# vicpc00/td-vc-gan

Hardware: AMD Instinct MI355X
Metric: audio-seconds/sec (G+D train step, stage-1) (higher is better)
Workload: dtype f32 (fp32 storage and accumulation everywhere; FiLM cond_var.2 forward and weight-grad as split-bf16 x6 products -- three exact bf16 pieces per operand, six piece products on the bf16 MFMA, fp32 accumulate: fp32-level accuracy; every other kernel exact-fp32 MFMA)

## Files before the change

### td-vc-gan_amd/csrc/conv_common.h

```cpp
#pragma once
#include <hip/hip_runtime.h>
#include <stdint.h>
#include <mutex>

#define TDVC_BIG_LDS_ONCE(k)                                                                                         \
  do {                                                                                                               \
    static std::once_flag f_;                                                                                        \
    std::call_once(f_, [&] { hipFuncSetAttribute(reinterpret_cast<const void*>(k), hipFuncAttributeMaxDynamicSharedMemorySize, 160 * 1024); }); \
  } while (0)
namespace tdvc {
extern int g_trace_on;
extern int g_force_tile;
extern int g_force_gemm_tile;
extern int g_force_generic;
extern int g_lds_cap;
extern int g_knob[9];
void trace_kernel(const void* fn);
}
#define TDVC_TRACE(k) do { if (tdvc::g_trace_on) tdvc::trace_kernel(reinterpret_cast<const void*>(k)); } while (0)

namespace tdvc {

enum { MODE_DIRECT = 0, MODE_DOWN = 1, MODE_UP = 2 };
enum { XF_NONE = 0, XF_LRELU = 1, XF_FILM_LRELU = 2, XF_MASK_LRELU = 3, XF_MASK_TANH = 4 };
enum { EPI_FWD = 0, EPI_MASK = 1, EPI_FILM = 2, EPI_PLAIN = 3 };
enum { POST_NONE = 0, POST_LRELU = 1, POST_TANH = 2 };

struct Xf {
  int kind; float slope; float scale;
  const float* aux; long aux_bs;
};

struct Opnd {
  const float* p; long bs; int T; int Cg; Xf xf;
};

struct GemmConvP {
  Opnd x;
  const float* w; long w_sg, w_sm, w_sc; int K; int tap_flip;
  int mode, s, d, pad, reflect, J;
  int R, Cred, Cc, N, groups, lo, span, XS, WS;
  int i0;
  int mirror_pad;
  int stage_rows;
  int chan_stage;
  int w_nat;
  int w_packed;
  float* y; long y_bs; int Ty; int Cy_g;
  int epi;
  const float* bias;
  const float* bias3;
  const float* res; long res_bs;
  int post; float post_slope; float out_scale;
  const float* add; long add_bs; float add_scale;
  const float* mx; long mx_bs; float m_slope;
  const float* gb; long gb_bs; float* dgb; long dgb_bs;
};

struct WgradP {
  Opnd a;
  Opnd x;
  int mode, s, d, pad, reflect, J, K;
  int R, Cred, N, groups, lo, span, NTc, XS, AS;
  int i0;
  int ntiles;
  float* slab; long slab_stride;
  long w_sg, w_sm, w_sc;
};

// ... 51 lines not shown
__device__ __forceinline__ void tile_commit(const RegTile<NV>& t, const RegTile<NV>* a, const RegTile<NV>* c, const Xf& xf,
                                            float* dst, int XS, int nvalid, int nrows, int span, int ebase, int tid) {
  typedef float f32x2_t __attribute__((ext_vector_type(2)));
  const int nvec = span >> 2, total = nrows * nvec;
  const float inv = 1.0f / (float)nvec;
  const int kind = xf.kind;
  const float sl = xf.slope, sc = xf.scale;
#pragma unroll
  for (int i = 0; i < NV; ++i) {
    const int e = ebase + tid + i * 256;
    if (e >= total) continue;
    const int r = (int)(((float)e + 0.5f) * inv);
    const int vv = e - r * nvec;
    f32x4_t val = t.v[i];
    if (r < nvalid) {
      if (kind == XF_LRELU) {
#pragma unroll
        for (int q = 0; q < 4; ++q) val[q] = fmaxf(val[q], val[q] * sl);
      } else if (kind == XF_FILM_LRELU) {
#pragma unroll
        for (int q = 0; q < 4; ++q) { const float h = val[q] * (1.f + a->v[i][q]) + c->v[i][q]; val[q] = fmaxf(h, h * sl); }
      } else if (kind == XF_MASK_LRELU) {
#pragma unroll
        for (int q = 0; q < 4; ++q) val[q] = a->v[i][q] > 0.f ? val[q] : val[q] * sl;
      } else if (kind == XF_MASK_TANH) {
#pragma unroll
        for (int q = 0; q < 4; ++q) val[q] = val[q] * (1.f - a->v[i][q] * a->v[i][q]);
      }
      if (sc != 1.f) {
#pragma unroll
        for (int q = 0; q < 4; ++q) val[q] *= sc;
      }
    }
    f32x2_t* d2 = reinterpret_cast<f32x2_t*>(dst + r * XS + 4 * vv);
    d2[0] = (f32x2_t){val[0], val[1]};
    d2[1] = (f32x2_t){val[2], val[3]};
  }
}

typedef __amdgpu_buffer_rsrc_t srd_t;
typedef unsigned int u32x4_t __attribute__((ext_vector_type(4)));

__device__ __forceinline__ srd_t make_srd(const float* base, int bytes) {
  const uintptr_t a = reinterpret_cast<uintptr_t>(base);
  const unsigned lo = __builtin_amdgcn_readfirstlane((unsigned)(a & 0xffffffffu));
  const unsigned hi = __builtin_amdgcn_readfirstlane((unsigned)(a >> 32));
  const int nb = __builtin_amdgcn_readfirstlane(bytes > 0 ? bytes : 0);
  float* ub = reinterpret_cast<float*>(((uintptr_t)hi << 32) | lo);
  return __builtin_amdgcn_make_buffer_rsrc(ub, 0, nb, 0x00020000);
}
__device__ __forceinline__ f32x4_t buf_load4(srd_t rs, int voff) {
  return __builtin_bit_cast(f32x4_t, __builtin_amdgcn_raw_buffer_load_b128(rs, voff, 0, 0));
}

template <int NV>
__device__ __forceinline__ void tile_issue(RegTile<NV>& t, const float* base, int rowstride, int nvalid, int nrows, int span,
                                           int cvalid, int ebase, int tid, int vlo, int vhi) {
  const int nvec = span >> 2, total = nrows * nvec;
  const float inv = 1.0f / (float)nvec;
  const srd_t rs = make_srd(base, nvalid > 0 ? ((nvalid - 1) * rowstride + cvalid) * 4 : 0);
#pragma unroll
  for (int i = 0; i < NV; ++i) {
    const int e = ebase + tid + i * 256;
    const int r = (int)(((float)e + 0.5f) * inv);
    const int vv = e - r * nvec;
    t.v[i] = buf_load4(rs, (e < total && r < nvalid && 4 * vv < cvalid && vv >= vlo && vv < vhi) ? (r * rowstride + 4 * vv) * 4 : 0x7f000000);
  }
}

struct RowWalk { int voff, loff, gstep, lstep, nk; bool active; };

__device__ __forceinline__ int walk_opaque(int n) { asm volatile("" : "+s"(n)); return n; }

__device__ __forceinline__ RowWalk make_walk(int tid, int nvec, int rp, int rowstride, int ls, int q0, int T) {
  RowWalk w;
  const int rsub = (int)(((float)tid + 0.5f) * (1.0f / (float)nvec));
  const int vv = tid - rsub * nvec;
  const int q = q0 + 4 * vv;
  w.active = rsub < rp;
  w.voff = (w.active && q >= 0 && q < T) ? (rsub * rowstride + q) * 4 : 0x7f000000;
  w.nk = T - q < 4 ? T - q : 4;
  w.loff = rsub * ls + 4 * vv;
  w.gstep = rp * rowstride * 4;
  w.lstep = rp * ls;
  return w;
}

template <int NP>
__device__ __forceinline__ void walk_issue(RegTile<NP>& t, srd_t rs, const RowWalk& w, int np) {
  int vo = w.voff;
#pragma unroll
  for (int i = 0; i < NP; ++i) {
    if (i < walk_opaque(np)) { t.v[i] = buf_load4(rs, vo); vo += w.gstep; }
  }
}

template <int NP>
__device__ __forceinline__ void walk_commit_act(RegTile<NP>& t, const RowWalk& w, int np, float* lds, float slope, float scale, bool tail = false) {
  if (!w.active) return;
  const int base = w.loff;
#pragma unroll
  for (int i = 0; i < NP; ++i) {
    if (i < walk_opaque(np)) {
      f32x4_t o;
#pragma unroll
      for (int q = 0; q < 4; ++q) { const float v = t.v[i][q]; o[q] = fmaxf(v, v * slope); }
// ... 144 lines not shown
```

### td-vc-gan_amd/csrc/conv_lean.h

```cpp
#pragma once
#include <hip/hip_runtime.h>

namespace tdvc {

enum { LXF_ACT = 0, LXF_FILM = 1, LXF_MASK_LRELU = 2, LXF_MASK_TANH = 3, LXF_COND = 4 };

struct LeanP {
  const float* x; const float* w; float* y;
  const float* bias; const float* bias3; const float* res; const float* add;
  const float* aux;
  const float* mx; const float* gb; float* dgb;
  int x_bs, y_bs, res_bs, add_bs, aux_bs, mx_bs, gb_bs, dgb_bs;
  int T, Cin, Cout, Cw, K, d, pad, flip, reflect, mirror;
  int Cc, span, lo, i0, XS, WS;
  int xrp, xnp, wrp, wnp;
  int post;
  const float* cw; const float* k3; float* cv0;
  int cw_stride, Cv, cv0_bs, ES;
  unsigned* sbits; const unsigned* mbits;
  int sb_bs, mb_bs;
  int swz;
  int one_ahead;
  int fold, seg, Bn;
  int vec;
  float slope, in_scale, out_scale, add_scale, m_slope;
};

hipError_t launch_conv_lean(LeanP p, int B, int xfk, int epi, hipStream_t st);
hipError_t launch_conv_lean_cond(LeanP p, int B, hipStream_t st);

}
```

### td-vc-gan_amd/csrc/conv_lean.hip

```cpp
#include "conv_common.h"
#include "conv_lean.h"

PROF_DEFINE(tdvc_debug_lean_prof)

namespace tdvc {

typedef float f32x4 __attribute__((ext_vector_type(4)));




template <int XFK>
__device__ __forceinline__ float lean_xform(const LeanP& p, float v, int b, int c, int q) {
  if (XFK == LXF_ACT) { v = fmaxf(v, v * p.slope); }
  else {
    const float* a = p.aux + (long)b * p.aux_bs + (long)c * p.T + q;
    if (XFK == LXF_FILM) { const float h = v * (1.f + a[0]) + a[(long)p.Cin * p.T]; v = fmaxf(h, h * p.slope); }
    else if (XFK == LXF_MASK_LRELU) { v = a[0] > 0.f ? v : v * p.slope; }
    else { v = v * (1.f - a[0] * a[0]); }
  }
  return v * p.in_scale;
}

template <int XFK>
__device__ __forceinline__ float lean_fetch(const LeanP& p, int b, int c, int q) {
  if (p.reflect) { if (q < 0) q = -q; else if (q >= p.T) q = 2 * (p.T - 1) - q; }
  if (q < 0 || q >= p.T) return 0.f;
  return lean_xform<XFK>(p, p.x[(long)b * p.x_bs + (long)c * p.T + q], b, c, q);
}

#ifndef LEAN_OCC_SMALL
#define LEAN_OCC_SMALL 4
#endif
constexpr int lean_min_blocks(int m_rep, int n_rep, int wm, int xfk) {
  if (m_rep == 1 && n_rep == 4 && wm == 1 && xfk == LXF_ACT) return 5;
  return m_rep * n_rep >= 9 ? 2 : ((m_rep * n_rep >= 8 || (wm == 4 && xfk == LXF_FILM)) ? 3 : LEAN_OCC_SMALL);
}
#ifndef LEAN_RING_1
#define LEAN_RING_1 2
#endif
#ifndef LEAN_RING_2
#define LEAN_RING_2 2
#endif
constexpr int lean_ring_depth(int m_rep, int n_rep) { return m_rep * n_rep == 1 ? LEAN_RING_1 : (m_rep * n_rep == 2 ? LEAN_RING_2 : 0); }
template <int M_REP, int N_REP, int WM, int WN, int XFK, int EPI, bool FOLD = false>
__global__ __launch_bounds__(256, lean_min_blocks(M_REP, N_REP, WM, XFK)) void conv_lean_kernel(const LeanP p) {
  extern __shared__ __attribute__((aligned(16))) float smem[];
  constexpr int MT = 16 * M_REP * WM, NT = 16 * N_REP * WN;
  constexpr int XVP = (M_REP >= 9 || NT <= 64) ? 4 : (MT >= 32 ? 12 : 6);
  constexpr int WVP = MT >= 48 ? 10 : (MT >= 32 ? 6 : 4);
  float* xs = smem;
  float* ws = smem + p.xnp * p.xrp * p.XS;
  constexpr int WX = 25;
  float* es = ws + p.wnp * p.wrp * p.WS;
  float* wx = es + p.Cv * p.ES;

  const int tid = threadIdx.x, lane = tid & 63, wave = tid >> 6;
  const int wm = wave / WN, wn = wave % WN;
  const int ln = lane & 15, kq = lane >> 4;
  int bx = blockIdx.x, by = blockIdx.y, bz = blockIdx.z;
  if (p.swz) {
    const int gx = gridDim.x, gy = gridDim.y;
    const int nwg = gx * gy * gridDim.z;
    const int orig = bx + gx * (by + gy * bz);
    const int q = nwg >> 3, r = nwg & 7, xcd = orig & 7;
    const int wg = (xcd < r ? xcd * (q + 1) : r * (q + 1) + (xcd - r) * q) + (orig >> 3);
    by = wg % gy;
    const int t = wg / gy;
    bx = t % gx; bz = t / gx;
  }
  const int n0 = FOLD ? 0 : bx * NT, r0 = by * MT, b = FOLD ? bz * p.fold : bz;
  const int wcol0 = wn * 16 * N_REP, wrow0 = wm * 16 * M_REP;
  PROF_DECL

  f32x4 acc[M_REP][N_REP];
#pragma unroll
  for (int m = 0; m < M_REP; ++m)
#pragma unroll
    for (int n = 0; n < N_REP; ++n) acc[m][n] = (f32x4){0.f, 0.f, 0.f, 0.f};

  const int q0 = n0 + p.lo;
  const bool vec_ok = p.vec != 0;
  const bool interior = (XFK != LXF_COND) && (XFK == LXF_ACT || !p.reflect);
  const bool tail = (p.T & 3) != 0;
  const bool end_tile = q0 < 0 || q0 + p.span > p.T;
  const int jc = p.K * p.Cc;
  const float* xrow0 = p.x + (long)b * p.x_bs;
  const float* arow0 = (XFK != LXF_ACT && XFK != LXF_COND) ? p.aux + (long)b * p.aux_bs : nullptr;
  const float* wgrow = p.w + (long)r0 * p.Cw;
// ... 322 lines not shown
#pragma unroll
            for (int n = 0; n < N_REP; ++n) mbv[n] = mv[n] ? mb[n] : -(1 << 28);
            for (int j = 0; j < p.K; ++j) {
              const float* wp = w_lane + (p.flip ? p.K - 1 - j : j);
              const float* xp[N_REP]; bool ok[N_REP];
#pragma unroll
              for (int n = 0; n < N_REP; ++n) {
                const int idx = mbv[n] + j * p.d;
                ok[n] = (unsigned)idx < (unsigned)p.span;
                xp[n] = xs + kq * p.XS + (ok[n] ? idx : 0);
              }
              ring_run(csteps, [&](int slot) {
#pragma unroll
                for (int m = 0; m < M_REP; ++m) wv[slot][m] = wp[m * wrep];
#pragma unroll
                for (int n = 0; n < N_REP; ++n) { xv[slot][n] = *xp[n]; xp[n] += 4 * p.XS; }
                wp += 4 * p.K;
              }, [&](int slot) {
#pragma unroll
                for (int m = 0; m < M_REP; ++m)
#pragma unroll
                  for (int n = 0; n < N_REP; ++n)
                    acc[m][n] = __builtin_amdgcn_mfma_f32_16x16x4f32(ok[n] ? xv[slot][n] : 0.f, wv[slot][m], acc[m][n], 0, 0, 0);
              });
            }
            continue;
          }
        }
        for (int j = 0; j < p.K; ++j) {
          const float* wj = w_lane + (p.flip ? p.K - 1 - j : j);
          for (int cs = 0; cs < csteps; ++cs) {
            float wm_[M_REP], xm_[N_REP];
#pragma unroll
            for (int m = 0; m < M_REP; ++m) wm_[m] = wj[m * 16 * p.WS + cs * 4 * p.K];
#pragma unroll
            for (int n = 0; n < N_REP; ++n) {
              const int idx = mb[n] + j * p.d;
              const bool ok = mv[n] && idx >= 0 && idx < p.span;
              const float t = xs[(cs * 4 + kq) * p.XS + (ok ? idx : 0)];
              xm_[n] = ok ? t : 0.f;
            }
#pragma unroll
            for (int m = 0; m < M_REP; ++m)
#pragma unroll
              for (int n = 0; n < N_REP; ++n)
                acc[m][n] = __builtin_amdgcn_mfma_f32_16x16x4f32(xm_[n], wm_[m], acc[m][n], 0, 0, 0);
          }
        }
      }
    }
    PROF(5)
  }

  if (!vec_ok) {
#pragma unroll
    for (int m = 0; m < M_REP; ++m) {
      const int co = r0 + wrow0 + m * 16 + ln;
      if (co >= p.Cout) continue;
      const long ro = (long)co * p.T;
      const float bias = (EPI == EPI_FWD && p.bias) ? p.bias[co] : 0.f;
#pragma unroll
      for (int n = 0; n < N_REP; ++n) {
#pragma unroll
        for (int q = 0; q < 4; ++q) {
          const int t = n0 + wcol0 + n * 16 + kq * 4 + q;
          if (t >= p.T) continue;
          const long oi = ro + t;
          float v = acc[m][n][q];
          if (EPI == EPI_FWD) {
            v += bias;
            if (p.bias3) v += p.bias3[((long)b * p.Cout + co) * 3 + (t == 0 ? 0 : (t == p.T - 1 ? 2 : 1))];
            if (p.res) v += p.res[(long)b * p.res_bs + oi];
            if (p.post == POST_LRELU) v = fmaxf(v, v * p.m_slope);
            else if (p.post == POST_TANH) v = tanhf(v);
            v *= p.out_scale;
          } else if (EPI == EPI_MASK) {
            v = p.mx[(long)b * p.mx_bs + oi] > 0.f ? v : v * p.m_slope;
          } else if (EPI == EPI_FILM) {
            const float h = p.mx[(long)b * p.mx_bs + oi];
            const float* gp = p.gb + (long)b * p.gb_bs + oi;
            const float ga = gp[0], be = gp[(long)p.Cout * p.T];
            const float dh2 = (h * (1.f + ga) + be) > 0.f ? v : v * p.m_slope;
            float* dg = p.dgb + (long)b * p.dgb_bs + oi;
            dg[0] = dh2 * h; dg[(long)p.Cout * p.T] = dh2;
            v = dh2 * (1.f + ga);
          }
          if (p.add) v += p.add_scale * p.add[(long)b * p.add_bs + oi];
          p.y[(long)b * p.y_bs + oi] = v;
        }
      }
    }
    PROF(6)
    PROF_END
    return;
  }
  auto epi_store = [&](f32x4 v, const int co, const int t0, const float bias, const int b) -> f32x4 {
    const long oi = (long)co * p.T + t0;
    if (EPI == EPI_FWD) {
#pragma unroll
      for (int q = 0; q < 4; ++q) v[q] += bias;
      if (p.bias3) {
        const float* k3 = p.bias3 + ((long)b * p.Cout + co) * 3;
        const float mid = k3[1];
#pragma unroll
        for (int q = 0; q < 4; ++q) v[q] += mid;
        if (t0 == 0) v[0] += k3[0] - mid;
        if (t0 + 4 == p.T) v[3] += k3[2] - mid;
      }
      if (p.res) { const f32x4 r = *reinterpret_cast<const f32x4*>(p.res + (long)b * p.res_bs + oi); v += r; }
      if (p.post == POST_LRELU) {
#pragma unroll
        for (int q = 0; q < 4; ++q) v[q] = fmaxf(v[q], v[q] * p.m_slope);
      } else if (p.post == POST_TANH) {
#pragma unroll
        for (int q = 0; q < 4; ++q) v[q] = tanhf(v[q]);
      }
      v *= p.out_scale;
    } else if (EPI == EPI_MASK) {
      if (N_REP >= 2 && p.mbits) {
        const unsigned wbits = p.mbits[(long)b * p.mb_bs + (long)co * (p.T >> 5) + (t0 >> 5)] >> (t0 & 31);
#pragma unroll
        for (int q = 0; q < 4; ++q) v[q] = ((wbits >> q) & 1u) ? v[q] : v[q] * p.m_slope;
      } else {
        const f32x4 mm = *reinterpret_cast<const f32x4*>(p.mx + (long)b * p.mx_bs + oi);
#pragma unroll
        for (int q = 0; q < 4; ++q) v[q] = mm[q] > 0.f ? v[q] : v[q] * p.m_slope;
      }
    } else if (EPI == EPI_FILM) {
      const f32x4 h = *reinterpret_cast<const f32x4*>(p.mx + (long)b * p.mx_bs + oi);
      const float* gp = p.gb + (long)b * p.gb_bs + oi;
      const f32x4 ga = *reinterpret_cast<const f32x4*>(gp);
      const f32x4 be = *reinterpret_cast<const f32x4*>(gp + (long)p.Cout * p.T);
      f32x4 dga, dbe;
#pragma unroll
      for (int q = 0; q < 4; ++q) {
        const float h2 = h[q] * (1.f + ga[q]) + be[q];
        const float dh2 = h2 > 0.f ? v[q] : v[q] * p.m_slope;
        dga[q] = dh2 * h[q]; dbe[q] = dh2; v[q] = dh2 * (1.f + ga[q]);
      }
      float* dg = p.dgb + (long)b * p.dgb_bs + oi;
      *reinterpret_cast<f32x4*>(dg) = dga;
      *reinterpret_cast<f32x4*>(dg + (long)p.Cout * p.T) = dbe;
    }
    if (p.add) { const f32x4 a4 = *reinterpret_cast<const f32x4*>(p.add + (long)b * p.add_bs + oi); v += a4 * p.add_scale; }
    *reinterpret_cast<f32x4*>(p.y + (long)b * p.y_bs + oi) = v;
    return v;
  };
  auto sign_nibble = [](const f32x4& v, const int t0) -> unsigned {
    return ((v[0] > 0.f ? 1u : 0u) | (v[1] > 0.f ? 2u : 0u) | (v[2] > 0.f ? 4u : 0u) | (v[3] > 0.f ? 8u : 0u)) << (t0 & 31);
  };

#pragma unroll
  for (int m = 0; m < M_REP; ++m) {
    const int co = r0 + wrow0 + m * 16 + ln;
    if (co >= p.Cout) continue;
    float bias = 0.f;
    if (EPI == EPI_FWD && p.bias) bias = p.bias[co];
    unsigned sb_word = 0;
#pragma unroll
    for (int n = 0; n < N_REP; ++n) {
      int t0 = n0 + wcol0 + n * 16 + kq * 4, bb = b;
      if (FOLD) { const int sg = t0 / p.T; t0 -= sg * p.T; bb = b + sg; if (bb >= p.Bn) continue; }
      if (t0 >= p.T) continue;
      const f32x4 v = epi_store(acc[m][n], co, t0, bias, bb);
      if (EPI == EPI_FWD && N_REP >= 2 && p.sbits) {
        const unsigned h = sign_nibble(v, t0);
        sb_word = (n & 1) ? (sb_word | h) : h;
        if (n & 1) {
          unsigned w = sb_word;
          w |= (unsigned)__shfl_xor((int)w, 16);
          w |= (unsigned)__shfl_xor((int)w, 32);
          if (kq == 0) p.sbits[(long)b * p.sb_bs + (long)co * (p.T >> 5) + (t0 >> 5)] = w;
        }
      }
    }
  }
  PROF(6)
  PROF_END
}

static inline void walk_geometry(int rows, int nvec, int* rp, int* np) {
  *rp = nvec <= 256 ? 256 / nvec : 0;
  if (*rp > rows) *rp = rows;
  *np = *rp ? (rows + *rp - 1) / *rp : 1 << 20;
}

template <int M_REP, int N_REP, int WM, int WN, int XFK, int EPI, bool FOLD = false>
static hipError_t lean_launch3(const LeanP& p, int B, hipStream_t st) {
  constexpr int MT = 16 * M_REP * WM, NT = 16 * N_REP * WN;
  auto k = conv_lean_kernel<M_REP, N_REP, WM, WN, XFK, EPI, FOLD>;
  TDVC_BIG_LDS_ONCE(k); TDVC_TRACE(k);
  dim3 grid(FOLD ? 1 : (p.T + NT - 1) / NT, (p.Cout + MT - 1) / MT, FOLD ? (B + p.fold - 1) / p.fold : B);
  LeanP q = p; q.swz = g_knob[0] && (long)grid.x * grid.y * grid.z >= 16;
  q.one_ahead = g_knob[8] != 0;
  const size_t lds = (size_t)(p.xnp * p.xrp * p.XS + p.wnp * p.wrp * p.WS) * sizeof(float);
  hipLaunchKernelGGL(k, grid, dim3(256), lds, st, q);
  return hipGetLastError();
}

template <int M_REP, int N_REP, int WM, int WN>
static hipError_t lean_launch_fold(const LeanP& p, int B, int xfk, int epi, hipStream_t st) {
  if (xfk == LXF_ACT && epi == EPI_FWD) return lean_launch3<M_REP, N_REP, WM, WN, LXF_ACT, EPI_FWD, true>(p, B, st);
  if (xfk == LXF_ACT && epi == EPI_PLAIN) return lean_launch3<M_REP, N_REP, WM, WN, LXF_ACT, EPI_PLAIN, true>(p, B, st);
  if (xfk == LXF_MASK_LRELU && epi == EPI_PLAIN) return lean_launch3<M_REP, N_REP, WM, WN, LXF_MASK_LRELU, EPI_PLAIN, true>(p, B, st);
  return hipErrorNotSupported;
}

template <int M_REP, int N_REP, int WM, int WN>
static hipError_t lean_launch2(const LeanP& p, int B, int xfk, int epi, hipStream_t st) {
  if (xfk == LXF_ACT && epi == EPI_FWD) return lean_launch3<M_REP, N_REP, WM, WN, LXF_ACT, EPI_FWD>(p, B, st);
  if (xfk == LXF_FILM && epi == EPI_FWD) return lean_launch3<M_REP, N_REP, WM, WN, LXF_FILM, EPI_FWD>(p, B, st);
  if (xfk == LXF_ACT && epi == EPI_MASK) return lean_launch3<M_REP, N_REP, WM, WN, LXF_ACT, EPI_MASK>(p, B, st);
  if (xfk == LXF_ACT && epi == EPI_FILM) return lean_launch3<M_REP, N_REP, WM, WN, LXF_ACT, EPI_FILM>(p, B, st);
  if (xfk == LXF_ACT && epi == EPI_PLAIN) return lean_launch3<M_REP, N_REP, WM, WN, LXF_ACT, EPI_PLAIN>(p, B, st);
  if (xfk == LXF_MASK_LRELU && epi == EPI_PLAIN) return lean_launch3<M_REP, N_REP, WM, WN, LXF_MASK_LRELU, EPI_PLAIN>(p, B, st);
  return hipErrorNotSupported;
}

hipError_t launch_conv_lean_cond(LeanP p, int B, hipStream_t st) {
  if ((p.T & 3) || !p.vec || p.K != 3 || p.d != 1 || p.pad != 1 || p.Cv * 3 > 24) return hipErrorNotSupported;
  const int MT = p.Cout <= 32 ? 32 : 64, NT = 256;
  p.mirror = 0; p.flip = 0; p.reflect = 0;
  const int first = -p.pad;
  const int lo = -4;
  p.lo = lo; p.i0 = first - lo;
  p.span = ((NT + (p.K - 1) * p.d - p.pad - lo) + 3) / 4 * 4;
  p.XS = ((p.span + 15) / 32) * 32 + 16;
  p.ES = ((p.span + 15) / 16) * 16 + 4;
  int Cc = 32;
  auto geom = [&](int cc) {
    p.Cc = cc; p.WS = p.K * cc + 2;
    p.xrp = cc; p.xnp = 1;
    walk_geometry(MT, p.K * cc / 4, &p.wrp, &p.wnp);
    return (size_t)(cc * p.XS + p.wnp * p.wrp * p.WS + p.Cv * p.ES + cc * 25) * sizeof(float);
  };
  size_t lds = geom(Cc);
  if (lds > (size_t)(g_lds_cap > 0 ? g_lds_cap : 80 * 1024) || p.wnp > (MT >= 48 ? 10 : 6)) lds = geom(Cc = 16);
  dim3 grid((p.T + NT - 1) / NT, (p.Cout + MT - 1) / MT, B);
  p.swz = g_knob[0] && (long)grid.x * grid.y * grid.z >= 16;
  if (MT == 32) {
    auto k = conv_lean_kernel<2, 4, 1, 4, LXF_COND, EPI_FWD>;
    TDVC_BIG_LDS_ONCE(k); TDVC_TRACE(k);
    hipLaunchKernelGGL(k, grid, dim3(256), lds, st, p);
  } else {
    auto k = conv_lean_kernel<4, 4, 1, 4, LXF_COND, EPI_FWD>;
    TDVC_BIG_LDS_ONCE(k); TDVC_TRACE(k);
    hipLaunchKernelGGL(k, grid, dim3(256), lds, st, p);
  }
  return hipGetLastError();
}

hipError_t launch_conv_lean(LeanP p, int B, int xfk, int epi, hipStream_t st) {
  const bool combo = (xfk == LXF_ACT) || (xfk == LXF_FILM && epi == EPI_FWD) || (xfk == LXF_MASK_LRELU && epi == EPI_PLAIN);
  if (!combo) return hipErrorNotSupported;
  struct Cand { int MT, NT, cfg; };
  static const Cand cands[] = {{64, 256, 2}, {48, 256, 5}, {32, 256, 1}, {64, 64, 4}, {32, 64, 6}, {16, 256, 0}, {16, 64, 3}};
  static const Cand tall = {144, 64, 7};
  const int R = p.Cout;
  int MT = 16, NT = 64, cfg = 3;
  for (const Cand& c : cands) {
    if (c.MT > 16 && R <= 16) continue;
    if (c.MT > 32 && R <= 32) continue;
    if (c.MT == 48 && !(R % 64 != 0 && (R + 47) / 48 * 48 < (R + 63) / 64 * 64)) continue;
    if (c.MT == 64 && c.NT == 256 && (R % 64 != 0 && (R + 47) / 48 * 48 < (R + 63) / 64 * 64)) continue;
    if (c.NT == 256 && p.T <= 80) continue;
    const long blocks = (long)((R + c.MT - 1) / c.MT) * ((p.T + c.NT - 1) / c.NT) * B;
    MT = c.MT; NT = c.NT; cfg = c.cfg;
    if (blocks >= (c.cfg == 4 ? 1024 : 512)) break;
  }
  if ((long)p.Cin * p.K <= 48 && p.T > 80 && p.mirror == 0) { MT = 16; NT = 256; cfg = 0; }
  if ((long)p.Cin * p.K <= 224 && p.T > 80 && (R >= 128 || R == 32)) { MT = 16; NT = 256; cfg = 0; }
  if (g_force_tile >= 0) {
    for (const Cand& c : cands)
      if (c.cfg == g_force_tile) { MT = c.MT; NT = c.NT; cfg = c.cfg; }
    if (g_force_tile == tall.cfg) { MT = tall.MT; NT = tall.NT; cfg = tall.cfg; }
  }
  if (p.sbits || p.mbits) {
    if (!p.vec || (p.T & 31) || p.T <= 80) return hipErrorNotSupported;
    if (cfg == 3 || cfg == tall.cfg) { MT = 16; NT = 256; cfg = 0; }
  }
  const int first = -p.pad;
  int lo = -p.pad - p.mirror;
  lo = -(((-lo) + 3) / 4 * 4);
  const int hi = (p.K - 1) * p.d - p.pad + p.mirror;
  p.lo = lo; p.i0 = first - lo;
  p.span = ((NT + hi - lo) + 3) / 4 * 4;
  p.fold = 1; p.seg = 0; p.Bn = B;
  const bool fold_combo = (xfk == LXF_ACT && (epi == EPI_FWD || epi == EPI_PLAIN)) || (xfk == LXF_MASK_LRELU && epi == EPI_PLAIN);
  if (g_knob[4] == 0 && g_force_tile < 0 && NT == 64 && R >= 32 && (p.T == 16 || p.T == 32) && p.Cin % 16 == 0 && B >= 64 / p.T && p.vec && !p.reflect && p.mirror == 0 && fold_combo &&
      !p.sbits && !p.mbits && (!p.aux || p.aux_bs == p.x_bs) && (long)(64 / p.T) * p.x_bs < (1L << 28)) {
    p.fold = 64 / p.T;
    p.seg = ((p.T + hi - lo) + 3) / 4 * 4;
    p.span = p.fold * p.seg;
    const long nb64 = (long)((R + 63) / 64) * ((B + p.fold - 1) / p.fold);
    if (nb64 >= 1024) { MT = 64; cfg = 4; } else { MT = 32; cfg = 6; }
  }
  p.XS = ((p.span + 15) / 32) * 32 + 16;
  const int xvp = (MT >= 144 || NT <= 64) ? 4 : (MT >= 32 ? 12 : 6), wvp = MT >= 48 ? 10 : (MT >= 32 ? 6 : 4);
  const size_t lds_cap = g_lds_cap > 0 ? (size_t)g_lds_cap : (size_t)((cfg == 4 ? 40 : 52) * 1024);
  int Cc = 0;
  const int cc_cap = (MT == 16 && p.Cin >= 256) ? 64 : 32;
  for (int cc = 4; cc <= cc_cap && cc <= ((p.Cin + 3) / 4) * 4; cc += 4) {
    int xrp, xnp, wrp, wnp;
    walk_geometry(cc, p.span / 4, &xrp, &xnp);
    walk_geometry(MT, p.K * cc / 4, &wrp, &wnp);
    const size_t lds = (size_t)(xnp * xrp * p.XS + wnp * wrp * (p.K * cc + 2)) * 4;
    if (lds > lds_cap || wnp > wvp || (xfk == LXF_ACT && xnp > xvp)) continue;
    if (p.fold > 1 && p.Cin % cc) continue;
    Cc = cc; p.xrp = xrp; p.xnp = xnp; p.wrp = wrp; p.wnp = wnp;
  }
  if (!Cc) return hipErrorNotSupported;
  p.Cc = Cc;
  p.WS = p.K * Cc + 2;
  if (p.fold > 1) return cfg == 4 ? lean_launch_fold<1, 4, 4, 1>(p, B, xfk, epi, st) : lean_launch_fold<1, 2, 2, 2>(p, B, xfk, epi, st);
  switch (cfg) {
    case 0: return lean_launch2<1, 4, 1, 4>(p, B, xfk, epi, st);
    case 1: return lean_launch2<2, 4, 1, 4>(p, B, xfk, epi, st);
    case 2: return lean_launch2<4, 4, 1, 4>(p, B, xfk, epi, st);
    case 3: return lean_launch2<1, 1, 1, 4>(p, B, xfk, epi, st);
    case 5: return lean_launch2<3, 4, 1, 4>(p, B, xfk, epi, st);
    case 6: return lean_launch2<1, 2, 2, 2>(p, B, xfk, epi, st);
    case 7: return lean_launch2<9, 1, 1, 4>(p, B, xfk, epi, st);
    default: return lean_launch2<1, 4, 4, 1>(p, B, xfk, epi, st);
  }
}

}
```

### td-vc-gan_amd/csrc/misc_kernels.hip

```cpp
#include "../../include/tdvc.h"
#include "api_util.h"
#include "conv_common.h"
#include <math.h>
#include <stdlib.h>
#include <string.h>

static thread_local char g_err[256] = "";
int tdvc_fail(int code, const char* msg) {
  snprintf(g_err, sizeof(g_err), "%s", msg ? msg : "");
  return code;
}
extern "C" const char* tdvc_last_error(void) { return g_err; }
extern "C" int tdvc_version(void) { return 200; }

#include <cxxabi.h>
#include <mutex>
#include <set>
#include <string>
namespace tdvc {
int g_trace_on = 0;
int g_force_tile = -1;
int g_force_gemm_tile = -1;
int g_lds_cap = 0;
int g_knob[9] = {0, 0, 0, 0, 0, 0, 0, 0, 0};
static std::mutex g_trace_mu;
static std::set<std::string> g_trace_names;
void trace_kernel(const void* fn) {
  const char* mangled = hipKernelNameRefByPtr(fn, nullptr);
  std::string name;
  if (mangled) {
    int status = 0;
    char* dem = abi::__cxa_demangle(mangled, nullptr, nullptr, &status);
    name = (status == 0 && dem) ? dem : mangled;
    free(dem);
  } else {
    char buf[32]; snprintf(buf, sizeof(buf), "kernel@%p", fn); name = buf;
  }
  std::lock_guard<std::mutex> lk(g_trace_mu);
  g_trace_names.insert(name);
}
}
extern "C" void tdvc_debug_force_tile(int cfg) { tdvc::g_force_tile = cfg; }
extern "C" void tdvc_debug_force_gemm_tile(int cfg) { tdvc::g_force_gemm_tile = cfg; }
extern "C" void tdvc_debug_lds_cap(int bytes) { tdvc::g_lds_cap = bytes; }
extern "C" void tdvc_debug_knob(int which, int value) { if (which >= 0 && which < 9) tdvc::g_knob[which] = value; }
namespace tdvc {
__global__ __launch_bounds__(256) void poison_lds_kernel(unsigned word, int nwords, unsigned* sink) {
  extern __shared__ __attribute__((aligned(16))) float smem[];
  unsigned* u = reinterpret_cast<unsigned*>(smem);
  for (int i = threadIdx.x; i < nwords; i += 256) u[i] = word;
  __syncthreads();
  unsigned acc = 0;
  for (int i = threadIdx.x; i < nwords; i += 256) acc ^= u[i];
  if (acc == 0x12345u && sink) sink[0] = acc;
}
}
extern "C" int tdvc_debug_poison_lds(uint32_t word, void* stream) {
  auto k = tdvc::poison_lds_kernel;
  TDVC_BIG_LDS_ONCE(k);
  hipLaunchKernelGGL(k, dim3(4096), dim3(256), 80 * 1024, (hipStream_t)stream, (unsigned)word, 80 * 1024 / 4, (unsigned*)nullptr);
  TDVC_CHECK_LAUNCH();
  return TDVC_OK;
}
namespace tdvc { __global__ void pmc_marker_kernel(int*) {} }
extern "C" int tdvc_debug_marker(void* stream) {
  hipLaunchKernelGGL(tdvc::pmc_marker_kernel, dim3(1), dim3(64), 0, (hipStream_t)stream, (int*)nullptr);
  TDVC_CHECK_LAUNCH();
  return TDVC_OK;
}
extern "C" void tdvc_debug_trace(int on) {
  std::lock_guard<std::mutex> lk(tdvc::g_trace_mu);
  if (on == 1) tdvc::g_trace_names.clear();
  tdvc::g_trace_on = on ? 1 : 0;
}
extern "C" size_t tdvc_debug_trace_dump(char* buf, size_t cap) {
  std::lock_guard<std::mutex> lk(tdvc::g_trace_mu);
  std::string all;
  for (const std::string& n : tdvc::g_trace_names) { all += n; all += '\n'; }
  if (buf && cap) { const size_t n = all.size() < cap - 1 ? all.size() : cap - 1; memcpy(buf, all.data(), n); buf[n] = 0; }
  return all.size() + 1;
}

namespace {

__device__ __forceinline__ float wave_sum(float v) {
#pragma unroll
  for (int o = 32; o > 0; o >>= 1) v += __shfl_xor(v, o);
  return v;
}

__device__ __forceinline__ float block_sum(float v, float* sh ) {
  v = wave_sum(v);
  __syncthreads();
  if ((threadIdx.x & 63) == 0) sh[threadIdx.x >> 6] = v;
  __syncthreads();
  float r = 0.f;
  const int nw = (blockDim.x + 63) >> 6;
  for (int i = 0; i < nw; ++i) r += sh[i];
// ... 938 lines not shown
```

Baseline: 313.6.

## Batch epilogue loads through buffer descriptors and specialize epilogue variants

Rewrites the lean conv kernel epilogue so that each group of output rows issues all of its auxiliary loads (residual, mask, FiLM gamma/beta, add, bias) first, then computes. Out-of-range accesses go through raw buffer loads and stores with bounds-checked descriptors instead of per-element branches. The epilogue is instantiated at compile time for vector vs scalar, add, mask bits and post-activation, which removes runtime branches and extends the vectorised path to folded tiles. The previous epilogue remains available behind a new debug knob. In exchange, register pressure and code size go up, which could hurt occupancy.

```diff
diff --git a/td-vc-gan_amd/csrc/conv_common.h b/td-vc-gan_amd/csrc/conv_common.h
--- a/td-vc-gan_amd/csrc/conv_common.h
+++ b/td-vc-gan_amd/csrc/conv_common.h
@@ -14,7 +14,7 @@
 extern int g_force_gemm_tile;
 extern int g_force_generic;
 extern int g_lds_cap;
-extern int g_knob[9];
+extern int g_knob[10];
 void trace_kernel(const void* fn);
 }
 #define TDVC_TRACE(k) do { if (tdvc::g_trace_on) tdvc::trace_kernel(reinterpret_cast<const void*>(k)); } while (0)
@@ -172,6 +172,15 @@
 __device__ __forceinline__ f32x4_t buf_load4(srd_t rs, int voff) {
   return __builtin_bit_cast(f32x4_t, __builtin_amdgcn_raw_buffer_load_b128(rs, voff, 0, 0));
 }
+__device__ __forceinline__ float buf_load1(srd_t rs, int voff) {
+  return __builtin_bit_cast(float, __builtin_amdgcn_raw_buffer_load_b32(rs, voff, 0, 0));
+}
+__device__ __forceinline__ void buf_store4(srd_t rs, int voff, f32x4_t v) {
+  __builtin_amdgcn_raw_buffer_store_b128(__builtin_bit_cast(u32x4_t, v), rs, voff, 0, 0);
+}
+__device__ __forceinline__ void buf_store1(srd_t rs, int voff, float v) {
+  __builtin_amdgcn_raw_buffer_store_b32(__builtin_bit_cast(unsigned, v), rs, voff, 0, 0);
+}
 
 template <int NV>
 __device__ __forceinline__ void tile_issue(RegTile<NV>& t, const float* base, int rowstride, int nvalid, int nrows, int span,
diff --git a/td-vc-gan_amd/csrc/conv_lean.h b/td-vc-gan_amd/csrc/conv_lean.h
--- a/td-vc-gan_amd/csrc/conv_lean.h
+++ b/td-vc-gan_amd/csrc/conv_lean.h
@@ -21,6 +21,7 @@
   int sb_bs, mb_bs;
   int swz;
   int one_ahead;
+  int old_epi;
   int fold, seg, Bn;
   int vec;
   float slope, in_scale, out_scale, add_scale, m_slope;
diff --git a/td-vc-gan_amd/csrc/conv_lean.hip b/td-vc-gan_amd/csrc/conv_lean.hip
--- a/td-vc-gan_amd/csrc/conv_lean.hip
+++ b/td-vc-gan_amd/csrc/conv_lean.hip
@@ -1,5 +1,7 @@
 #include "conv_common.h"
 #include "conv_lean.h"
+#include <algorithm>
+#include <type_traits>
 
 PROF_DEFINE(tdvc_debug_lean_prof)
 
@@ -35,6 +37,15 @@
 constexpr int lean_min_blocks(int m_rep, int n_rep, int wm, int xfk) {
   if (m_rep == 1 && n_rep == 4 && wm == 1 && xfk == LXF_ACT) return 5;
   return m_rep * n_rep >= 9 ? 2 : ((m_rep * n_rep >= 8 || (wm == 4 && xfk == LXF_FILM)) ? 3 : LEAN_OCC_SMALL);
+}
+constexpr int lean_epi_rows(int m_rep, int n_rep, int epi) {
+  int r = 16 / (n_rep * (epi == EPI_FILM ? 4 : 2));
+  r = r < 1 ? 1 : (r > m_rep ? m_rep : r);
+  while (m_rep % r) --r;
+  return r;
+}
+constexpr int lean_epi_cols(int m_rep, int n_rep, int wm, int xfk, int epi) {
+  return (m_rep == 1 && n_rep == 4 && wm == 1 && xfk == LXF_ACT && epi == EPI_FILM) ? 2 : n_rep;
 }
 #ifndef LEAN_RING_1
 #define LEAN_RING_1 2
@@ -463,41 +474,124 @@
     PROF(5)
   }
 
-  if (!vec_ok) {
-#pragma unroll
-    for (int m = 0; m < M_REP; ++m) {
-      const int co = r0 + wrow0 + m * 16 + ln;
-      if (co >= p.Cout) continue;
-      const long ro = (long)co * p.T;
-      const float bias = (EPI == EPI_FWD && p.bias) ? p.bias[co] : 0.f;
-#pragma unroll
-      for (int n = 0; n < N_REP; ++n) {
-#pragma unroll
-        for (int q = 0; q < 4; ++q) {
-          const int t = n0 + wcol0 + n * 16 + kq * 4 + q;
-          if (t >= p.T) continue;
-          const long oi = ro + t;
-          float v = acc[m][n][q];
-          if (EPI == EPI_FWD) {
-            v += bias;
-            if (p.bias3) v += p.bias3[((long)b * p.Cout + co) * 3 + (t == 0 ? 0 : (t == p.T - 1 ? 2 : 1))];
-            if (p.res) v += p.res[(long)b * p.res_bs + oi];
-            if (p.post == POST_LRELU) v = fmaxf(v, v * p.m_slope);
-            else if (p.post == POST_TANH) v = tanhf(v);
-            v *= p.out_scale;
-          } else if (EPI == EPI_MASK) {
-            v = p.mx[(long)b * p.mx_bs + oi] > 0.f ? v : v * p.m_slope;
-          } else if (EPI == EPI_FILM) {
-            const float h = p.mx[(long)b * p.mx_bs + oi];
-            const float* gp = p.gb + (long)b * p.gb_bs + oi;
-            const float ga = gp[0], be = gp[(long)p.Cout * p.T];
-            const float dh2 = (h * (1.f + ga) + be) > 0.f ? v : v * p.m_slope;
-            float* dg = p.dgb + (long)b * p.dgb_bs + oi;
-            dg[0] = dh2 * h; dg[(long)p.Cout * p.T] = dh2;
-            v = dh2 * (1.f + ga);
-          }
-          if (p.add) v += p.add_scale * p.add[(long)b * p.add_bs + oi];
-          p.y[(long)b * p.y_bs + oi] = v;
+  auto sign_nibble = [](const f32x4& v, const int t0) -> unsigned {
+    return ((v[0] > 0.f ? 1u : 0u) | (v[1] > 0.f ? 2u : 0u) | (v[2] > 0.f ? 4u : 0u) | (v[3] > 0.f ? 8u : 0u)) << (t0 & 31);
+  };
+  if (p.old_epi) {
+    if (!vec_ok) {
+#pragma unroll
+      for (int m = 0; m < M_REP; ++m) {
+        const int co = r0 + wrow0 + m * 16 + ln;
+        if (co >= p.Cout) continue;
+        const long ro = (long)co * p.T;
+        const float bias = (EPI == EPI_FWD && p.bias) ? p.bias[co] : 0.f;
+#pragma unroll
+        for (int n = 0; n < N_REP; ++n) {
+#pragma unroll
+          for (int q = 0; q < 4; ++q) {
+            const int t = n0 + wcol0 + n * 16 + kq * 4 + q;
+            if (t >= p.T) continue;
+            const long oi = ro + t;
+            float v = acc[m][n][q];
+            if (EPI == EPI_FWD) {
+              v += bias;
+              if (p.bias3) v += p.bias3[((long)b * p.Cout + co) * 3 + (t == 0 ? 0 : (t == p.T - 1 ? 2 : 1))];
+              if (p.res) v += p.res[(long)b * p.res_bs + oi];
+              if (p.post == POST_LRELU) v = fmaxf(v, v * p.m_slope);
+              else if (p.post == POST_TANH) v = tanhf(v);
+              v *= p.out_scale;
+            } else if (EPI == EPI_MASK) {
+              v = p.mx[(long)b * p.mx_bs + oi] > 0.f ? v : v * p.m_slope;
+            } else if (EPI == EPI_FILM) {
+              const float h = p.mx[(long)b * p.mx_bs + oi];
+              const float* gp = p.gb + (long)b * p.gb_bs + oi;
+              const float ga = gp[0], be = gp[(long)p.Cout * p.T];
+              const float dh2 = (h * (1.f + ga) + be) > 0.f ? v : v * p.m_slope;
+              float* dg = p.dgb + (long)b * p.dgb_bs + oi;
+              dg[0] = dh2 * h; dg[(long)p.Cout * p.T] = dh2;
+              v = dh2 * (1.f + ga);
+            }
+            if (p.add) v += p.add_scale * p.add[(long)b * p.add_bs + oi];
+            p.y[(long)b * p.y_bs + oi] = v;
+          }
+        }
+      }
+    } else {
+      auto epi_store = [&](f32x4 v, const int co, const int t0, const float bias, const int b) -> f32x4 {
+        const long oi = (long)co * p.T + t0;
+        if (EPI == EPI_FWD) {
+#pragma unroll
+          for (int q = 0; q < 4; ++q) v[q] += bias;
+          if (p.bias3) {
+            const float* k3 = p.bias3 + ((long)b * p.Cout + co) * 3;
+            const float mid = k3[1];
+#pragma unroll
+            for (int q = 0; q < 4; ++q) v[q] += mid;
+            if (t0 == 0) v[0] += k3[0] - mid;
+            if (t0 + 4 == p.T) v[3] += k3[2] - mid;
+          }
+          if (p.res) { const f32x4 r = *reinterpret_cast<const f32x4*>(p.res + (long)b * p.res_bs + oi); v += r; }
+          if (p.post == POST_LRELU) {
+#pragma unroll
+            for (int q = 0; q < 4; ++q) v[q] = fmaxf(v[q], v[q] * p.m_slope);
+          } else if (p.post == POST_TANH) {
+#pragma unroll
+            for (int q = 0; q < 4; ++q) v[q] = tanhf(v[q]);
+          }
+          v *= p.out_scale;
+        } else if (EPI == EPI_MASK) {
+          if (N_REP >= 2 && p.mbits) {
+            const unsigned wbits = p.mbits[(long)b * p.mb_bs + (long)co * (p.T >> 5) + (t0 >> 5)] >> (t0 & 31);
+#pragma unroll
+            for (int q = 0; q < 4; ++q) v[q] = ((wbits >> q) & 1u) ? v[q] : v[q] * p.m_slope;
+          } else {
+            const f32x4 mm = *reinterpret_cast<const f32x4*>(p.mx + (long)b * p.mx_bs + oi);
+#pragma unroll
+            for (int q = 0; q < 4; ++q) v[q] = mm[q] > 0.f ? v[q] : v[q] * p.m_slope;
+          }
+        } else if (EPI == EPI_FILM) {
+          const f32x4 h = *reinterpret_cast<const f32x4*>(p.mx + (long)b * p.mx_bs + oi);
+          const float* gp = p.gb + (long)b * p.gb_bs + oi;
+          const f32x4 ga = *reinterpret_cast<const f32x4*>(gp);
+          const f32x4 be = *reinterpret_cast<const f32x4*>(gp + (long)p.Cout * p.T);
+          f32x4 dga, dbe;
+#pragma unroll
+          for (int q = 0; q < 4; ++q) {
+            const float h2 = h[q] * (1.f + ga[q]) + be[q];
+            const float dh2 = h2 > 0.f ? v[q] : v[q] * p.m_slope;
+            dga[q] = dh2 * h[q]; dbe[q] = dh2; v[q] = dh2 * (1.f + ga[q]);
+          }
+          float* dg = p.dgb + (long)b * p.dgb_bs + oi;
+          *reinterpret_cast<f32x4*>(dg) = dga;
+          *reinterpret_cast<f32x4*>(dg + (long)p.Cout * p.T) = dbe;
+        }
+        if (p.add) { const f32x4 a4 = *reinterpret_cast<const f32x4*>(p.add + (long)b * p.add_bs + oi); v += a4 * p.add_scale; }
+        *reinterpret_cast<f32x4*>(p.y + (long)b * p.y_bs + oi) = v;
+        return v;
+      };
+#pragma unroll
+      for (int m = 0; m < M_REP; ++m) {
+        const int co = r0 + wrow0 + m * 16 + ln;
+        if (co >= p.Cout) continue;
+        float bias = 0.f;
+        if (EPI == EPI_FWD && p.bias) bias = p.bias[co];
+        unsigned sb_word = 0;
+#pragma unroll
+        for (int n = 0; n < N_REP; ++n) {
+          int t0 = n0 + wcol0 + n * 16 + kq * 4, bb = b;
+          if (FOLD) { const int sg = t0 / p.T; t0 -= sg * p.T; bb = b + sg; if (bb >= p.Bn) continue; }
+          if (t0 >= p.T) continue;
+          const f32x4 v = epi_store(acc[m][n], co, t0, bias, bb);
+          if (EPI == EPI_FWD && N_REP >= 2 && p.sbits) {
+            const unsigned h = sign_nibble(v, t0);
+            sb_word = (n & 1) ? (sb_word | h) : h;
+            if (n & 1) {
+              unsigned w = sb_word;
+              w |= (unsigned)__shfl_xor((int)w, 16);
+              w |= (unsigned)__shfl_xor((int)w, 32);
+              if (kq == 0) p.sbits[(long)b * p.sb_bs + (long)co * (p.T >> 5) + (t0 >> 5)] = w;
+            }
+          }
         }
       }
     }
@@ -505,86 +599,167 @@
     PROF_END
     return;
   }
-  auto epi_store = [&](f32x4 v, const int co, const int t0, const float bias, const int b) -> f32x4 {
-    const long oi = (long)co * p.T + t0;
-    if (EPI == EPI_FWD) {
-#pragma unroll
-      for (int q = 0; q < 4; ++q) v[q] += bias;
-      if (p.bias3) {
-        const float* k3 = p.bias3 + ((long)b * p.Cout + co) * 3;
-        const float mid = k3[1];
-#pragma unroll
-        for (int q = 0; q < 4; ++q) v[q] += mid;
-        if (t0 == 0) v[0] += k3[0] - mid;
-        if (t0 + 4 == p.T) v[3] += k3[2] - mid;
-      }
-      if (p.res) { const f32x4 r = *reinterpret_cast<const f32x4*>(p.res + (long)b * p.res_bs + oi); v += r; }
-      if (p.post == POST_LRELU) {
-#pragma unroll
-        for (int q = 0; q < 4; ++q) v[q] = fmaxf(v[q], v[q] * p.m_slope);
-      } else if (p.post == POST_TANH) {
-#pragma unroll
-        for (int q = 0; q < 4; ++q) v[q] = tanhf(v[q]);
-      }
-      v *= p.out_scale;
-    } else if (EPI == EPI_MASK) {
-      if (N_REP >= 2 && p.mbits) {
-        const unsigned wbits = p.mbits[(long)b * p.mb_bs + (long)co * (p.T >> 5) + (t0 >> 5)] >> (t0 & 31);
-#pragma unroll
-        for (int q = 0; q < 4; ++q) v[q] = ((wbits >> q) & 1u) ? v[q] : v[q] * p.m_slope;
-      } else {
-        const f32x4 mm = *reinterpret_cast<const f32x4*>(p.mx + (long)b * p.mx_bs + oi);
-#pragma unroll
-        for (int q = 0; q < 4; ++q) v[q] = mm[q] > 0.f ? v[q] : v[q] * p.m_slope;
-      }
-    } else if (EPI == EPI_FILM) {
-      const f32x4 h = *reinterpret_cast<const f32x4*>(p.mx + (long)b * p.mx_bs + oi);
-      const float* gp = p.gb + (long)b * p.gb_bs + oi;
-      const f32x4 ga = *reinterpret_cast<const f32x4*>(gp);
-      const f32x4 be = *reinterpret_cast<const f32x4*>(gp + (long)p.Cout * p.T);
-      f32x4 dga, dbe;
-#pragma unroll
-      for (int q = 0; q < 4; ++q) {
-        const float h2 = h[q] * (1.f + ga[q]) + be[q];
-        const float dh2 = h2 > 0.f ? v[q] : v[q] * p.m_slope;
-        dga[q] = dh2 * h[q]; dbe[q] = dh2; v[q] = dh2 * (1.f + ga[q]);
-      }
-      float* dg = p.dgb + (long)b * p.dgb_bs + oi;
-      *reinterpret_cast<f32x4*>(dg) = dga;
-      *reinterpret_cast<f32x4*>(dg + (long)p.Cout * p.T) = dbe;
+  constexpr int EB = lean_epi_rows(M_REP, N_REP, EPI), NB = lean_epi_cols(M_REP, N_REP, WM, XFK, EPI);
+  constexpr int OOR = 0x7f000000;
+  const int ct = p.Cout * p.T;
+  const int nsamp = FOLD ? min(p.fold, p.Bn - b) : 1;
+  const bool has_res = EPI == EPI_FWD && p.res != nullptr, has_b3 = EPI == EPI_FWD && p.bias3 != nullptr;
+  auto srd_of = [&](const float* base, int bs, bool has) __attribute__((always_inline)) {
+    return make_srd(has ? base + (long)b * bs : nullptr, has ? ((nsamp - 1) * bs + ct) * 4 : 0);
+  };
+  auto epilogue = [&](auto VEC_, auto ADD_, auto BITS_, auto POST_) __attribute__((always_inline)) {
+    constexpr bool VEC = decltype(VEC_)::value, ADD = decltype(ADD_)::value, BITS = decltype(BITS_)::value;
+    constexpr int POST = decltype(POST_)::value;
+    constexpr bool MX = (EPI == EPI_MASK && !BITS) || EPI == EPI_FILM;
+    const srd_t sy = srd_of(p.y, p.y_bs, true), sadd = srd_of(p.add, p.add_bs, ADD), sres = srd_of(p.res, p.res_bs, has_res);
+    const srd_t smx = srd_of(p.mx, p.mx_bs, MX);
+    const srd_t sga = srd_of(p.gb, p.gb_bs, EPI == EPI_FILM), sbe = srd_of(p.gb + ct, p.gb_bs, EPI == EPI_FILM);
+    const srd_t sdg = srd_of(p.dgb, p.dgb_bs, EPI == EPI_FILM), sdb = srd_of(p.dgb + ct, p.dgb_bs, EPI == EPI_FILM);
+    const srd_t sbit = make_srd(BITS ? reinterpret_cast<const float*>(p.mbits + (long)b * p.mb_bs) : nullptr, BITS ? p.Cout * (p.T >> 5) * 4 : 0);
+    const srd_t sbias = make_srd(p.bias, (EPI == EPI_FWD && p.bias) ? p.Cout * 4 : 0);
+    const srd_t sb3 = make_srd(has_b3 ? p.bias3 + (long)b * p.Cout * 3 : nullptr, has_b3 ? nsamp * p.Cout * 12 : 0);
+    auto ld = [&](const srd_t s, const int o, const int t0) __attribute__((always_inline)) -> f32x4 {
+      if constexpr (VEC) return buf_load4(s, o);
+      else {
+        f32x4 r;
+#pragma unroll
+        for (int q = 0; q < 4; ++q) r[q] = buf_load1(s, (o != OOR && t0 + q < p.T) ? o + 4 * q : OOR);
+        return r;
+      }
+    };
+    auto st = [&](const srd_t s, const int o, const int t0, const f32x4 v) __attribute__((always_inline)) {
+      if constexpr (VEC) buf_store4(s, o, v);
+      else {
+#pragma unroll
+        for (int q = 0; q < 4; ++q) buf_store1(s, (o != OOR && t0 + q < p.T) ? o + 4 * q : OOR, v[q]);
+      }
+    };
+#pragma unroll
+    for (int m0 = 0; m0 < M_REP; m0 += EB) {
+      int tt[N_REP], sg[N_REP], off[EB][N_REP];
+      bool ok[EB][N_REP];
+      f32x4 vmx[EB][N_REP], vadd[EB][N_REP], vres[EB][N_REP], vga[EB][N_REP], vbe[EB][N_REP];
+      unsigned wb[EB][N_REP];
+      float bias[EB], k3v[EB][FOLD ? N_REP : 1][3];
+      auto at = [&](int mi, int n, int bs) __attribute__((always_inline)) { return FOLD ? (ok[mi][n] ? off[mi][n] + sg[n] * bs * 4 : OOR) : off[mi][n]; };
+#pragma unroll
+      for (int n = 0; n < N_REP; ++n) {
+        tt[n] = n0 + wcol0 + n * 16 + kq * 4; sg[n] = 0;
+        if (FOLD) { sg[n] = tt[n] / p.T; tt[n] -= sg[n] * p.T; }
+      }
+#pragma unroll
+      for (int nb = 0; nb < N_REP; nb += NB) {
+#pragma unroll
+        for (int mi = 0; mi < EB; ++mi) {
+          const int co = r0 + wrow0 + (m0 + mi) * 16 + ln;
+          if (EPI == EPI_FWD && nb == 0) {
+            bias[mi] = buf_load1(sbias, co * 4);
+#pragma unroll
+            for (int s = 0; s < (FOLD ? N_REP : 1); ++s)
+#pragma unroll
+              for (int e = 0; e < 3; ++e)
+                k3v[mi][s][e] = buf_load1(sb3, (co < p.Cout && sg[s] < nsamp) ? ((sg[s] * p.Cout + co) * 3 + e) * 4 : OOR);
+          }
+#pragma unroll
+          for (int n = nb; n < nb + NB; ++n) {
+            ok[mi][n] = co < p.Cout && tt[n] < p.T && (!FOLD || sg[n] < nsamp);
+            off[mi][n] = ok[mi][n] ? (co * p.T + tt[n]) * 4 : OOR;
+            if (EPI == EPI_FWD) vres[mi][n] = ld(sres, at(mi, n, p.res_bs), tt[n]);
+            if constexpr (BITS) wb[mi][n] = __builtin_bit_cast(unsigned, buf_load1(sbit, ok[mi][n] ? (co * (p.T >> 5) + (tt[n] >> 5)) * 4 : OOR));
+            if constexpr (MX) vmx[mi][n] = ld(smx, at(mi, n, p.mx_bs), tt[n]);
+            if (EPI == EPI_FILM) { vga[mi][n] = ld(sga, at(mi, n, p.gb_bs), tt[n]); vbe[mi][n] = ld(sbe, at(mi, n, p.gb_bs), tt[n]); }
+            if constexpr (ADD) vadd[mi][n] = ld(sadd, at(mi, n, p.add_bs), tt[n]);
+          }
+        }
+#pragma unroll
+        for (int mi = 0; mi < EB; ++mi) {
+          const int co = r0 + wrow0 + (m0 + mi) * 16 + ln;
+          unsigned sb_word = 0;
+#pragma unroll
+          for (int n = nb; n < nb + NB; ++n) {
+            const int t0 = tt[n];
+            f32x4 v = acc[m0 + mi][n];
+            if (EPI == EPI_FWD) {
+#pragma unroll
+              for (int q = 0; q < 4; ++q) v[q] += bias[mi];
+              const float* k3 = k3v[mi][FOLD ? n : 0];
+              if constexpr (VEC) {
+                const float mid = k3[1];
+#pragma unroll
+                for (int q = 0; q < 4; ++q) v[q] = has_b3 ? v[q] + mid : v[q];
+                v[0] = (has_b3 && t0 == 0) ? v[0] + (k3[0] - mid) : v[0];
+                v[3] = (has_b3 && t0 + 4 == p.T) ? v[3] + (k3[2] - mid) : v[3];
+              } else {
+#pragma unroll
+                for (int q = 0; q < 4; ++q) v[q] = has_b3 ? v[q] + (t0 + q == 0 ? k3[0] : (t0 + q == p.T - 1 ? k3[2] : k3[1])) : v[q];
+              }
+#pragma unroll
+              for (int q = 0; q < 4; ++q) v[q] = has_res ? v[q] + vres[mi][n][q] : v[q];
+              if constexpr (POST == POST_LRELU) {
+#pragma unroll
+                for (int q = 0; q < 4; ++q) v[q] = fmaxf(v[q], v[q] * p.m_slope);
+              } else if constexpr (POST == POST_TANH) {
+#pragma unroll
+                for (int q = 0; q < 4; ++q) v[q] = tanhf(v[q]);
+              }
+              v *= p.out_scale;
+            } else if (EPI == EPI_MASK) {
+              if constexpr (BITS) {
+                const unsigned wbits = wb[mi][n] >> (t0 & 31);
+#pragma unroll
+                for (int q = 0; q < 4; ++q) v[q] = ((wbits >> q) & 1u) ? v[q] : v[q] * p.m_slope;
+              } else {
+                const f32x4 mm = vmx[mi][n];
+#pragma unroll
+                for (int q = 0; q < 4; ++q) v[q] = mm[q] > 0.f ? v[q] : v[q] * p.m_slope;
+              }
+            } else if (EPI == EPI_FILM) {
+              const f32x4 h = vmx[mi][n], ga = vga[mi][n], be = vbe[mi][n];
+              f32x4 dga, dbe;
+#pragma unroll
+              for (int q = 0; q < 4; ++q) {
+                const float h2 = h[q] * (1.f + ga[q]) + be[q];
+                const float dh2 = h2 > 0.f ? v[q] : v[q] * p.m_slope;
+                dga[q] = dh2 * h[q]; dbe[q] = dh2; v[q] = dh2 * (1.f + ga[q]);
+              }
+              st(sdg, at(mi, n, p.dgb_bs), t0, dga);
+              st(sdb, at(mi, n, p.dgb_bs), t0, dbe);
+            }
+            if constexpr (ADD) v += vadd[mi][n] * p.add_scale;
+            st(sy, at(mi, n, p.y_bs), t0, v);
+            if (EPI == EPI_FWD && N_REP >= 2 && p.sbits) {
+              const unsigned h = sign_nibble(v, t0);
+              sb_word = (n & 1) ? (sb_word | h) : h;
+              if (n & 1) {
+                unsigned w = sb_word;
+                w |= (unsigned)__shfl_xor((int)w, 16);
+                w |= (unsigned)__shfl_xor((int)w, 32);
+                if (kq == 0 && ok[mi][n]) p.sbits[(long)b * p.sb_bs + (long)co * (p.T >> 5) + (t0 >> 5)] = w;
+              }
+            }
+          }
+        }
+      }
     }
-    if (p.add) { const f32x4 a4 = *reinterpret_cast<const f32x4*>(p.add + (long)b * p.add_bs + oi); v += a4 * p.add_scale; }
-    *reinterpret_cast<f32x4*>(p.y + (long)b * p.y_bs + oi) = v;
-    return v;
   };
-  auto sign_nibble = [](const f32x4& v, const int t0) -> unsigned {
-    return ((v[0] > 0.f ? 1u : 0u) | (v[1] > 0.f ? 2u : 0u) | (v[2] > 0.f ? 4u : 0u) | (v[3] > 0.f ? 8u : 0u)) << (t0 & 31);
+  constexpr std::false_type NO{};
+  constexpr std::true_type YES{};
+  constexpr std::integral_constant<int, POST_NONE> P0{};
+  auto by_kind = [&](auto V, auto A) __attribute__((always_inline)) {
+    if constexpr (EPI == EPI_FWD) {
+      if (p.post == POST_LRELU) epilogue(V, A, NO, std::integral_constant<int, POST_LRELU>{});
+      else if (p.post == POST_TANH) epilogue(V, A, NO, std::integral_constant<int, POST_TANH>{});
+      else epilogue(V, A, NO, P0);
+    } else if constexpr (EPI == EPI_MASK && N_REP >= 2 && decltype(V)::value) {
+      if (p.mbits) epilogue(V, A, YES, P0); else epilogue(V, A, NO, P0);
+    } else {
+      epilogue(V, A, NO, P0);
+    }
   };
-
-#pragma unroll
-  for (int m = 0; m < M_REP; ++m) {
-    const int co = r0 + wrow0 + m * 16 + ln;
-    if (co >= p.Cout) continue;
-    float bias = 0.f;
-    if (EPI == EPI_FWD && p.bias) bias = p.bias[co];
-    unsigned sb_word = 0;
-#pragma unroll
-    for (int n = 0; n < N_REP; ++n) {
-      int t0 = n0 + wcol0 + n * 16 + kq * 4, bb = b;
-      if (FOLD) { const int sg = t0 / p.T; t0 -= sg * p.T; bb = b + sg; if (bb >= p.Bn) continue; }
-      if (t0 >= p.T) continue;
-      const f32x4 v = epi_store(acc[m][n], co, t0, bias, bb);
-      if (EPI == EPI_FWD && N_REP >= 2 && p.sbits) {
-        const unsigned h = sign_nibble(v, t0);
-        sb_word = (n & 1) ? (sb_word | h) : h;
-        if (n & 1) {
-          unsigned w = sb_word;
-          w |= (unsigned)__shfl_xor((int)w, 16);
-          w |= (unsigned)__shfl_xor((int)w, 32);
-          if (kq == 0) p.sbits[(long)b * p.sb_bs + (long)co * (p.T >> 5) + (t0 >> 5)] = w;
-        }
-      }
-    }
+  if (FOLD || vec_ok) {
+    if (p.add) by_kind(YES, YES); else by_kind(YES, NO);
+  } else if constexpr (!FOLD) {
+    if (p.add) by_kind(NO, YES); else by_kind(NO, NO);
   }
   PROF(6)
   PROF_END
@@ -604,6 +779,7 @@
   dim3 grid(FOLD ? 1 : (p.T + NT - 1) / NT, (p.Cout + MT - 1) / MT, FOLD ? (B + p.fold - 1) / p.fold : B);
   LeanP q = p; q.swz = g_knob[0] && (long)grid.x * grid.y * grid.z >= 16;
   q.one_ahead = g_knob[8] != 0;
+  q.old_epi = g_knob[9] != 0;
   const size_t lds = (size_t)(p.xnp * p.xrp * p.XS + p.wnp * p.wrp * p.WS) * sizeof(float);
   hipLaunchKernelGGL(k, grid, dim3(256), lds, st, q);
   return hipGetLastError();
@@ -649,6 +825,7 @@
   if (lds > (size_t)(g_lds_cap > 0 ? g_lds_cap : 80 * 1024) || p.wnp > (MT >= 48 ? 10 : 6)) lds = geom(Cc = 16);
   dim3 grid((p.T + NT - 1) / NT, (p.Cout + MT - 1) / MT, B);
   p.swz = g_knob[0] && (long)grid.x * grid.y * grid.z >= 16;
+  p.old_epi = g_knob[9] != 0;
   if (MT == 32) {
     auto k = conv_lean_kernel<2, 4, 1, 4, LXF_COND, EPI_FWD>;
     TDVC_BIG_LDS_ONCE(k); TDVC_TRACE(k);
@@ -699,7 +876,8 @@
   p.fold = 1; p.seg = 0; p.Bn = B;
   const bool fold_combo = (xfk == LXF_ACT && (epi == EPI_FWD || epi == EPI_PLAIN)) || (xfk == LXF_MASK_LRELU && epi == EPI_PLAIN);
   if (g_knob[4] == 0 && g_force_tile < 0 && NT == 64 && R >= 32 && (p.T == 16 || p.T == 32) && p.Cin % 16 == 0 && B >= 64 / p.T && p.vec && !p.reflect && p.mirror == 0 && fold_combo &&
-      !p.sbits && !p.mbits && (!p.aux || p.aux_bs == p.x_bs) && (long)(64 / p.T) * p.x_bs < (1L << 28)) {
+      !p.sbits && !p.mbits && (!p.aux || p.aux_bs == p.x_bs) && (long)(64 / p.T) * p.x_bs < (1L << 28) &&
+      (long)(64 / p.T) * std::max(p.y_bs, std::max(p.res ? p.res_bs : 0, p.add ? p.add_bs : 0)) < (1L << 28)) {
     p.fold = 64 / p.T;
     p.seg = ((p.T + hi - lo) + 3) / 4 * 4;
     p.span = p.fold * p.seg;
diff --git a/td-vc-gan_amd/csrc/misc_kernels.hip b/td-vc-gan_amd/csrc/misc_kernels.hip
--- a/td-vc-gan_amd/csrc/misc_kernels.hip
+++ b/td-vc-gan_amd/csrc/misc_kernels.hip
@@ -22,7 +22,7 @@
 int g_force_tile = -1;
 int g_force_gemm_tile = -1;
 int g_lds_cap = 0;
-int g_knob[9] = {0, 0, 0, 0, 0, 0, 0, 0, 0};
+int g_knob[10] = {0, 0, 0, 0, 0, 0, 0, 0, 0, 0};
 static std::mutex g_trace_mu;
 static std::set<std::string> g_trace_names;
 void trace_kernel(const void* fn) {
@@ -43,7 +43,7 @@
 extern "C" void tdvc_debug_force_tile(int cfg) { tdvc::g_force_tile = cfg; }
 extern "C" void tdvc_debug_force_gemm_tile(int cfg) { tdvc::g_force_gemm_tile = cfg; }
 extern "C" void tdvc_debug_lds_cap(int bytes) { tdvc::g_lds_cap = bytes; }
-extern "C" void tdvc_debug_knob(int which, int value) { if (which >= 0 && which < 9) tdvc::g_knob[which] = value; }
+extern "C" void tdvc_debug_knob(int which, int value) { if (which >= 0 && which < 10) tdvc::g_knob[which] = value; }
 namespace tdvc {
 __global__ __launch_bounds__(256) void poison_lds_kernel(unsigned word, int nwords, unsigned* sink) {
   extern __shared__ __attribute__((aligned(16))) float smem[];
```

New measurement: 316.8, median of 6. 1.01x the previous value.
